# gwlucastrig/gridfour

Hardware: AMD Instinct MI355X
Metric: encode+decode MB/s on int32 elevation tiles; bit-exact vs Java ref (higher is better)
Workload: dtype int32

## Files before the change

gridfour_amd/csrc/gvrs_decode.hip:

```cpp

#include <hip/hip_runtime.h>

#include <cstdlib>
#include <mutex>
#include <type_traits>

#include "gvrs_kernels.h"
#include "huff_build.h"

namespace {

constexpr int GF_K_SKIP = 0x7fff0001;
#ifndef GF_DEC_THREADS
#define GF_DEC_THREADS 256
#endif
#ifdef GF_DEC_VARIANT
#define GF_DEC_CAT2(a, b) a##b
#define GF_DEC_CAT(a, b) GF_DEC_CAT2(a, b)
#define gf_launch_huffman_decode GF_DEC_CAT(gf_launch_huffman_decode_t, GF_DEC_THREADS)
#define gf_huffman_decode_lds_per_wg GF_DEC_CAT(gf_huffman_decode_lds_per_wg_t, GF_DEC_THREADS)
#define gf_launch_huffman_decode_canon GF_DEC_CAT(gf_launch_huffman_decode_canon_t, GF_DEC_THREADS)
#endif
constexpr int DEC_THREADS = GF_DEC_THREADS;
constexpr int DEC_WAVES = DEC_THREADS / 64;
// ... 557 lines not shown
                if (cnt[i] & 3u) *reinterpret_cast<uint32_t *>(poolB + slot[i]) = lo[i];
                if (d[i] && cnt[i] > 4u * poolWords) S.poolOverflow = 1u;
            }
        }
#pragma unroll
        for (int i = 0; i < NCUR; i++)
            if (d[i]) { S.qs[qv[i]] = sPos[i]; S.qe[qv[i]] = a[i] - sh0; S.qn[qv[i]] = cnt[i]; }
    };
#ifdef GF_DIAG
    const uint32_t tBegin = (uint32_t)__builtin_amdgcn_s_memtime();
#endif
    {
        uint32_t qv[NCUR];
#pragma unroll
        for (int i = 0; i < NCUR; i++) qv[i] = tid + i * DEC_THREADS;
        runRound(true, qv);
    }
#ifdef GF_DIAG
    if (dbg && tid == 0) dbg[1] = (uint32_t)__builtin_amdgcn_s_memtime() - tBegin;
#endif
    for (uint32_t round = 1;; round++) {
        __syncthreads();
#ifdef GF_DIAG
        rounds++;
        if (dbg && tid == 0 && round == 1) dbg[3] = (uint32_t)__builtin_amdgcn_s_memtime() - tBegin;
#endif
        if (tid == 0) S.nRedo[(round + 1u) & 1u] = 0;
#pragma unroll
        for (int i = 0; i < NCUR; i++) {
            const uint32_t q = tid + i * DEC_THREADS;
            if (q > 0 && q < Q && S.qe[q - 1] != S.qs[q]) {
                const uint32_t slot = atomicAdd(&S.nRedo[round & 1u], 1u);
                if (slot < LIST_CAP) list[slot] = (uint16_t)q;
            }
        }
        __syncthreads();
        const uint32_t nList = min(S.nRedo[round & 1u], LIST_CAP);
        if (nList == 0) break;
#ifdef GF_DIAG
        listed += nList;
#endif
        uint32_t qv[NCUR];
#pragma unroll
        for (int i = 0; i < NCUR; i++) {
            const uint32_t slot = gf_wave_id() * (64u * NCUR) + (uint32_t)i * 64u + (tid & 63u);
            qv[i] = slot < nList ? list[slot] : 0xFFFFFFFFu;
        }
        runRound(false, qv);
    }
    uint32_t n[NCUR], sum = 0;
#pragma unroll
    for (int i = 0; i < NCUR; i++) {
        const uint32_t q = NCUR * tid + i;
        n[i] = q < Q ? S.qn[q] : 0u;
        sum += n[i];
    }
    uint32_t tot;
    uint32_t run = block_excl_scan(sum, S.waveSum, &tot);
#pragma unroll
    for (int i = 0; i < NCUR; i++) {
        const uint32_t q = NCUR * tid + i;
        if (q < Q) S.qn[q] = run;
        run += n[i];
    }
    if (tid == 0) S.chainTotal = tot;
#ifdef GF_DIAG
    if (dbg && tid == 0) { dbg[0] = rounds; dbg[DBG_LISTED] = listed; dbg[4] = (uint32_t)__builtin_amdgcn_s_memtime() - tBegin; }
#endif
    __syncthreads();
}

struct RCur {
    uint32_t pos, sh, r0, r1, r2, r3, r4, r5, r6, r7;
};
__device__ __forceinline__ void rcur_load(RCur &c, const uint32_t *__restrict__ base32, uint32_t nW, uint32_t sh0, uint32_t p)
{
    const uint32_t a = p + sh0, wi = a >> 5;
    c.pos = p;
    c.sh = a & 31u;
    if (wi + 8u <= nW) {
        const GfU4 x = *reinterpret_cast<const GfU4 *>(base32 + wi), y = *reinterpret_cast<const GfU4 *>(base32 + wi + 4);
        c.r0 = x.x; c.r1 = x.y; c.r2 = x.z; c.r3 = x.w;
        c.r4 = y.x; c.r5 = y.y; c.r6 = y.z; c.r7 = y.w;
    } else {
        const uint32_t last = nW - 1u;
        c.r0 = base32[min(wi, last)];
        c.r1 = base32[min(wi + 1u, last)];
        c.r2 = base32[min(wi + 2u, last)];
        c.r3 = base32[min(wi + 3u, last)];
        c.r4 = base32[min(wi + 4u, last)];
        c.r5 = base32[min(wi + 5u, last)];
        c.r6 = base32[min(wi + 6u, last)];
        c.r7 = base32[min(wi + 7u, last)];
    }
}
__device__ __forceinline__ void rcur_advance(RCur &c, uint32_t len)
{
    c.pos += len;
    const uint32_t sh = c.sh + len;
    const bool ge = sh >= 32u;
    c.r0 = ge ? c.r1 : c.r0;
    c.r1 = ge ? c.r2 : c.r1;
    c.r2 = ge ? c.r3 : c.r2;
    c.r3 = ge ? c.r4 : c.r3;
    c.r4 = ge ? c.r5 : c.r4;
    c.r5 = ge ? c.r6 : c.r5;
    c.r6 = ge ? c.r7 : c.r6;
    c.sh = sh & 31u;
}
constexpr uint32_t RCUR_BUDGET = 256u - 31u - 96u;

__device__ __forceinline__ void pool_to_m32(DecShared &S, const uint32_t *pool, uint32_t poolWords, uint32_t Q, uint32_t nM32, uint8_t *m32,
                                            uint32_t spare)
{
    const uint32_t tid = threadIdx.x;
    uint32_t *m32w = reinterpret_cast<uint32_t *>(m32);
#pragma unroll
    for (int i = 0; i < NCUR; i++) {
        const uint32_t q = tid + (uint32_t)i * DEC_THREADS;
        uint32_t base = 0, n = 0;
        if (q < Q) {
            base = S.qn[q];
            n = (q + 1u < Q ? S.qn[q + 1u] : S.chainTotal) - base;
            n = base < nM32 ? min(n, nM32 - base) : 0u;
        }
        const uint32_t *src = pool + (q < Q ? q : 0u);
        const uint32_t h = min(n, (0u - base) & 3u);
        const uint32_t nb = (n - h) >> 2, r = (n - h) & 3u;
        const uint32_t w0 = (base + h) >> 2;
        uint32_t tailWord = 0, first = 0;
        for (uint32_t c = 0; c < poolWords; c += 8u) {
            if (!__any(4u * c < n)) break;
            uint32_t w[9];
#pragma unroll
            for (uint32_t j = 0; j < 9u; j++) w[j] = c + j < poolWords ? src[(c + j) * Q] : 0u;
            if (c == 0u) first = w[0];
#pragma unroll
            for (uint32_t j = 0; j < 8u; j++) {
                const uint32_t k = c + j;
                const uint32_t out = __builtin_amdgcn_alignbyte(w[j + 1u], w[j], h);
                m32w[k < nb ? w0 + k : spare >> 2] = out;
                tailWord = k == nb ? out : tailWord;
            }
        }
#pragma unroll
        for (uint32_t j = 0; j < 3u; j++) {
            m32[j < h ? base + j : spare] = (uint8_t)(first >> (8u * j));
            m32[j < r ? base + h + 4u * nb + j : spare] = (uint8_t)(tailWord >> (8u * j));
        }
    }
}

template <int OWNER>
__device__ int32_t huffman_to_m32_fast(DecShared &S, const uint32_t *__restrict__ base32, uint32_t nW, uint32_t sh0,
                                       uint32_t *txt, uint32_t pkWords, const uint16_t *lut2, const unsigned long long *leafCodeG,
                                       uint32_t textStart, uint32_t endBit, uint32_t nM32, uint8_t *m32, uint32_t *dbg,
                                       const uint32_t warmBits, const int diagLimit = 0, uint32_t *pool = nullptr, uint32_t poolBytes = 0,
                                       uint32_t spareByte = 0)
{
    const uint32_t tid = threadIdx.x;
    int32_t status = GF_K_OK;
    const uint32_t textBits = endBit - textStart;
    uint32_t unit = (textBits + MAXQ - 1) / MAXQ;
    unit = max((uint32_t)GF_DEC_MIN_UNIT, (unit + 31u) & ~31u);
    const uint32_t Q = max(1u, (textBits + unit - 1) / unit);
    FastHuff H;
    H.S = &S;
    H.lut2 = lut2;
    H.leafCodeG = leafCodeG;
    H.l2bits = S.l2bits;
    H.nSub = S.nSub;
    uint16_t *cnt16 = reinterpret_cast<uint16_t *>(S.leafCode);
    static_assert(sizeof(S.leafCode) >= (sizeof(uint16_t) << LUT_BITS), "count table does not fit over leafCode");
    build_count_table(S, cnt16);
#ifdef GF_DIAG
    const uint32_t tStage = (uint32_t)__builtin_amdgcn_s_memtime();
#endif
    for (uint32_t i = tid + (uint32_t)EARLY_TXT * DEC_THREADS; i < pkWords + FAST_TEXT_PAD; i += DEC_THREADS) txt[i] = (i < pkWords && i < nW) ? base32[i] : 0u;
    __syncthreads();
#ifdef GF_DIAG
    if (dbg && tid == 0) dbg[2] = (uint32_t)__builtin_amdgcn_s_memtime() - tStage;
#endif
#ifdef GF_DIAG
    if (diagLimit == 7) return GF_K_SKIP;
#endif
    uint32_t poolWords = pool ? min(33u, (poolBytes / Q) >> 2) : 0u;
    poolWords = poolWords < 17u ? 0u : poolWords - 1u;
    fast_sync_pass<OWNER>(S, H, cnt16, txt, sh0, textStart, endBit, unit, Q, warmBits, dbg, poolWords ? pool : nullptr, poolWords);
#ifdef GF_DIAG
    if (diagLimit == 8) return GF_K_SKIP;
    if (dbg && tid == 0) dbg[-7] = (uint32_t)__builtin_amdgcn_s_memtime();
#else
    (void)dbg;
#endif
    if (S.chainTotal < nM32) status = GF_K_ERR_BOUNDS;
#ifdef GF_DEC_POOL_FORCE_OVERFLOW
    if (false) {
#else
    if (poolWords && !S.poolOverflow) {
#endif
        pool_to_m32(S, pool, poolWords, Q, nM32, m32, spareByte);
        if (status == GF_K_OK && S.chainTotal == nM32 && S.qe[Q - 1u] > endBit) status = GF_K_ERR_BOUNDS;
        __syncthreads();
        return status;
    }
    if (tid == 0) S.chainEnd = 0;
    __syncthreads();
    {
        bool d[NCUR];
        uint32_t k[NCUR], lim[NCUR];
        RCur c[NCUR];
#pragma unroll
        for (int i = 0; i < NCUR; i++) {
            const uint32_t q = tid + i * DEC_THREADS;
            d[i] = q < Q;
            k[i] = d[i] ? S.qn[q] : nM32;
            lim[i] = min(endBit, textStart + (q + 1) * unit);
            c[i].pos = d[i] ? S.qs[q] : endBit;
        }
        for (;;) {
            bool live[NCUR], anyLive = false;
#pragma unroll
            for (int i = 0; i < NCUR; i++) {
                live[i] = d[i] && c[i].pos < lim[i] && k[i] < nM32;
                anyLive = anyLive || live[i];
            }
            if (!__any(anyLive)) break;
            uint32_t blk[NCUR];
#pragma unroll
            for (int i = 0; i < NCUR; i++) {
                rcur_load(c[i], base32, nW, sh0, live[i] ? c[i].pos : 0u);
                if (!live[i]) c[i].pos = endBit;
                blk[i] = c[i].pos;
            }
            for (;;) {
                bool r[NCUR], any = false;
#pragma unroll
                for (int i = 0; i < NCUR; i++) {
                    r[i] = live[i] && c[i].pos < lim[i] && k[i] < nM32 && c[i].pos - blk[i] <= RCUR_BUDGET;
                    any = any || r[i];
                }
                if (!__any(any)) break;
                uint32_t x[NCUR], e[NCUR], anyLong = 0;
#pragma unroll
                for (int i = 0; i < NCUR; i++) {
                    x[i] = __builtin_amdgcn_alignbit(c[i].r1, c[i].r0, c[i].sh);
                    e[i] = S.lut[x[i] & ((1u << LUT_BITS) - 1u)];
                    anyLong |= e[i];
                }
                if (anyLong & 0x80000000u) {
#pragma unroll
                    for (int i = 0; i < NCUR; i++)
                        if (e[i] & 0x80000000u) e[i] = fh_resolve(H, e[i], x[i], c[i].r0, c[i].r1, c[i].r2, c[i].sh);
                }
#pragma unroll
                for (int i = 0; i < NCUR; i++) {
                    const uint32_t a1 = (e[i] >> 16) & 63u, t2 = e[i] >> 22;
                    const bool two = t2 != a1 && c[i].pos + a1 < lim[i] && nM32 - k[i] > 1u;
                    rcur_advance(c[i], r[i] ? (two ? t2 : a1) : 0u);
                    if (r[i]) {
                        m32[k[i]] = (uint8_t)e[i];
                        if (two) m32[k[i] + 1] = (uint8_t)(e[i] >> 8);
                        k[i] += two ? 2u : 1u;
                        if (k[i] == nM32) S.chainEnd = c[i].pos;
                    }
                }
            }
        }
    }
    __syncthreads();
    if (status == GF_K_OK && S.chainEnd > endBit) status = GF_K_ERR_BOUNDS;
    return status;
}


__device__ __forceinline__ int gf_writelane(int value, int lane, int old)
{
    return (int)(threadIdx.x & 63u) == lane ? value : old;
}

__device__ void parse_tree_wave(DecShared &S, uint32_t relBit, uint32_t absBit, uint32_t totalBits)
{
    const uint32_t lane = threadIdx.x & 63u;
    const uint32_t hw0 = S.head[lane];
    const uint32_t hw1 = lane < HEAD_WORDS - 64 ? S.head[64 + lane] : 0u;
    auto word = [&](uint32_t wi) -> uint32_t {
        if (wi >= HEAD_WORDS) return 0u;
        return (uint32_t)__builtin_amdgcn_readlane((int)(wi < 64 ? hw0 : hw1), (int)(wi & 63u));
    };
    const uint32_t fw = relBit >> 5, fs = relBit & 31u;
    uint64_t buf = (((uint64_t)word(fw + 1u) << 32) | word(fw)) >> fs;
    uint32_t have = 64u - fs, wnext = fw + 2u, bp = absBit;
    auto refill = [&]() {
        if (have <= 32) {
            buf |= (uint64_t)word(wnext) << have;
            have += 32;
            wnext++;
        }
    };
    auto take = [&](uint32_t nb) -> uint32_t {
        const uint32_t v = (uint32_t)buf & ((1u << nb) - 1u);
        buf >>= nb;
        have -= nb;
        bp += nb;
        return v;
    };
    const bool writer = lane == 0;
// ... 919 lines not shown

constexpr uint32_t BYTE_MAX_COLS = 256;
__device__ __forceinline__ bool byte_path_eligible(int model, uint32_t nR, uint32_t nC, uint32_t ldsM32Bytes)
{
    const uint32_t RB = (nR + DEC_WAVES - 1u) / DEC_WAVES;
    return model >= 1 && model <= 3 && nR >= 2u && nC >= 4u && nC <= BYTE_MAX_COLS && RB <= 255u && nR * nC + 8u <= ldsM32Bytes &&
           ((2u * nR + 3u) & ~3u) + (model == 3 ? (uint32_t)DEC_WAVES * ((nC + 3u) & ~3u) : 0u) <= SCR_WORDS;
}

template <int MODEL>
__device__ __forceinline__ void m32_bytes_rows(DecShared &S, const uint8_t *m32, const uint32_t seed, const uint32_t nR, const uint32_t nC,
                                               uint32_t *__restrict__ o)
{
    const uint32_t lane = threadIdx.x & 63u, wave = gf_wave_id();
    uint32_t *scr = reinterpret_cast<uint32_t *>(&S);
    uint32_t *col0 = scr, *d1s = scr + nR, *T = scr + ((2u * nR + 3u) & ~3u);
    const uint32_t TS = (nC + 3u) & ~3u;
    const uint32_t *m32w = reinterpret_cast<const uint32_t *>(m32);
    const uint32_t j0 = 4u * lane;
    const uint32_t jf = j0 < nC ? j0 : 0u;
    auto sx = [](uint32_t b) -> uint32_t { return (uint32_t)(int32_t)(int8_t)b; };
    if (wave == (uint32_t)DEC_WAVES - 1u) {
        uint32_t carry = seed;
        for (uint32_t rb = 0; rb < nR; rb += 64u) {
            const uint32_t r = rb + lane;
            uint32_t x = 0;
            if (r >= 1u && r < nR) x = sx(m32[MODEL == 3 ? nC - 2u + r : MODEL == 1 ? r * nC - 1u : 2u * r - 1u]);
            const uint32_t v = gf_wave_incl_scan(x) + carry;
            if (r < nR) col0[r] = v;
            carry = (uint32_t)__builtin_amdgcn_readlane((int)v, 63);
        }
    } else if (MODEL == 2 && wave == (uint32_t)DEC_WAVES - 2u) {
        for (uint32_t r = lane; r < nR; r += 64u) d1s[r] = sx(m32[2u * r]);
    }
    const uint32_t RB = (nR + DEC_WAVES - 1u) / DEC_WAVES;
    const uint32_t r0 = min(nR, wave * RB), r1 = min(nR, r0 + RB);
    const uint32_t rowStep = MODEL == 1 ? nC : MODEL == 2 ? nC - 2u : nC - 1u;
    auto rowAt = [&](uint32_t r) -> uint32_t {
        if (MODEL == 1) return r * nC - 1u;
        if (MODEL == 2) return 2u * nR - 1u + r * (nC - 2u) - 2u;
        return r ? nC + nR - 2u + (r - 1u) * (nC - 1u) - 1u : 0u - 1u;
    };
    auto fetch = [&](uint32_t a4) -> uint32_t {
        const uint32_t wi = a4 >> 2;
        return __builtin_amdgcn_alignbyte(m32w[wi], m32w[wi - 1u], a4 & 3u);
    };
    auto fetchRow0 = [&]() -> uint32_t { return __builtin_amdgcn_alignbyte(m32w[lane], lane ? m32w[lane - 1u] : 0u, 3u); };
    const bool peel = MODEL != 2 && r0 == 0u && r1 > 0u;
    const uint32_t keep0 = lane == 0u ? 0u : 0xFFFFFFFFu;
    uint32_t acc0 = 0, acc1 = 0, acc2 = 0, acc3 = 0;
    if (MODEL == 3) {
        if (wave + 1u < (uint32_t)DEC_WAVES && r1 > r0) {
            uint32_t ev = 0, od = 0;
            uint32_t r = r0;
            if (peel) {
                const uint32_t y = fetchRow0() ^ 0x80808080u;
                ev = y & 0x00FF00FFu;
                od = (y >> 8) & 0x00FF00FFu;
                r = 1u;
            }
            uint32_t a4 = rowAt(r) + jf + 4u;
            for (; r < r1; r++) {
                const uint32_t y = fetch(a4) ^ 0x80808080u;
                ev += y & 0x00FF00FFu;
                od += (y >> 8) & 0x00FF00FFu;
                a4 += rowStep;
            }
            const uint32_t bias = 128u * (r1 - r0);
            const uint32_t c0 = ((ev & 0xFFFFu) - bias) & keep0, c1 = (od & 0xFFFFu) - bias, c2 = (ev >> 16) - bias, c3 = (od >> 16) - bias;
            const uint32_t p1 = c0 + c1, p2 = p1 + c2, p3 = p2 + c3;
            const uint32_t ex = gf_wave_incl_scan(p3) - p3;
            if (j0 < TS) {
                uint32_t *Tw = T + wave * TS + j0;
                Tw[0] = ex + c0; Tw[1] = ex + p1; Tw[2] = ex + p2; Tw[3] = ex + p3;
            }
        }
    }
    __syncthreads();
    if (MODEL == 3 && j0 < TS) {
        for (uint32_t w = 0; w < wave; w++) {
            const uint32_t *Tw = T + w * TS + j0;
            acc0 += Tw[0]; acc1 += Tw[1]; acc2 += Tw[2]; acc3 += Tw[3];
        }
    }
    const uint32_t nFull = nC >> 2, rem = nC & 3u;
    const bool full = lane < nFull, part = lane == nFull && rem != 0u;
    struct Quad { uint32_t q0, q1, q2, q3; };
    auto sums = [&](uint32_t x, uint32_t left, uint32_t d1) -> Quad {
        const uint32_t v0 = sx(x) & keep0, v1 = MODEL == 2 ? sx(x >> 8) & keep0 : sx(x >> 8), v2 = sx(x >> 16), v3 = (uint32_t)((int32_t)x >> 24);
        const uint32_t p1 = v0 + v1, p2 = p1 + v2, p3 = p2 + v3;
        const uint32_t ex = gf_wave_incl_scan(p3) - p3;
        Quad q;
        if (MODEL == 2) {
            const uint32_t g1 = v0 + p1, g2 = g1 + p2, g3 = g2 + p3;
            const uint32_t t = g3 + 4u * ex;
            const uint32_t gx = gf_wave_incl_scan(t) - t;
            const uint32_t b = left + j0 * d1 + gx + ex;
            q.q0 = b + v0;
            q.q1 = b + d1 + ex + g1;
            q.q2 = b + 2u * (d1 + ex) + g2;
            q.q3 = b + 3u * (d1 + ex) + g3;
        } else if (MODEL == 3) {
            acc0 += ex + v0; acc1 += ex + p1; acc2 += ex + p2; acc3 += ex + p3;
            q.q0 = acc0 + left; q.q1 = acc1 + left; q.q2 = acc2 + left; q.q3 = acc3 + left;
        } else {
            const uint32_t b = left + ex;
            q.q0 = b + v0; q.q1 = b + p1; q.q2 = b + p2; q.q3 = b + p3;
        }
        return q;
    };
    auto put = [&](uint32_t r, const Quad &q) {
        uint32_t *dst = o + r * nC + j0;
        if (full) {
            GfU4 v;
            v.x = q.q0; v.y = q.q1; v.z = q.q2; v.w = q.q3;
            *reinterpret_cast<GfU4 *>(dst) = v;
        }
        if (part) {
            dst[0] = q.q0;
            if (rem >= 2u) dst[1] = q.q1;
            if (rem == 3u) dst[2] = q.q2;
        }
    };
    uint32_t r = r0;
    if (peel) {
        put(0u, sums(fetchRow0(), col0[0], 0u));
        r = 1u;
    }
    if (r < r1) {
        const uint32_t last = r1 - 1u;
        uint32_t a4 = rowAt(r) + jf + 4u, rB = min(r + 1u, last);
        uint32_t a4B = a4 + (rB - r) * rowStep;
        uint32_t xA = fetch(a4), leftA = col0[r], dA = MODEL == 2 ? d1s[r] : 0u;
        uint32_t xB = fetch(a4B), leftB = col0[rB], dB = MODEL == 2 ? d1s[rB] : 0u;
        for (; r < r1; r += 2u) {
            const uint32_t x0 = xA, l0 = leftA, e0 = dA, x1 = xB, l1 = leftB, e1 = dB;
            const uint32_t nA = min(r + 2u, last), nB = min(r + 3u, last);
            a4 += (nA - r) * rowStep;
            a4B = a4 + (nB - nA) * rowStep;
            xA = fetch(a4);
            leftA = col0[nA];
            xB = fetch(a4B);
            leftB = col0[nB];
            if (MODEL == 2) { dA = d1s[nA]; dB = d1s[nB]; }
            const Quad qa = sums(x0, l0, e0);
            const Quad qb = sums(x1, l1, e1);
            put(r, qa);
            if (r + 1u < r1) put(r + 1u, qb);
        }
    }
    __syncthreads();
}

template <class M32Ptr>
__device__ __forceinline__ void m32_bytes_to_tile(DecShared &S, M32Ptr m32, const int model, const uint32_t seed, const uint32_t nR,
                                                  const uint32_t nC, uint32_t *__restrict__ o)
{
    if (model == 3) m32_bytes_rows<3>(S, m32, seed, nR, nC, o);
    else if (model == 1) m32_bytes_rows<1>(S, m32, seed, nR, nC, o);
    else m32_bytes_rows<2>(S, m32, seed, nR, nC, o);
}

template <class M32Ptr>
__device__ int32_t huffman_serial_skips(DecShared &S, const uint32_t *__restrict__ base32, uint32_t nW, uint32_t sh0, uint32_t textStart,
                                        uint32_t endBit, uint32_t nM32, M32Ptr m32)
{
    const uint32_t tid = threadIdx.x, lane = tid & 63u;
    if (tid < 64u) {
        const uint32_t nLeaves = S.nLeaves;
        unsigned long long lc[4];
        uint32_t ll[4], ls[4];
#pragma unroll
        for (uint32_t j = 0; j < 4; j++) {
            const uint32_t i = lane + 64u * j;
            lc[j] = i < nLeaves ? S.leafCode[i] : 0ull;
            ll[j] = i < nLeaves ? (uint32_t)S.leafLen[i] : 0xFFu;
            ls[j] = i < nLeaves ? (uint32_t)S.leafSym[i] : 0u;
        }
        const uint32_t skipLen = GF_UNI(S.skipLen);
        const unsigned long long skipPath = ((unsigned long long)GF_UNI(S.skipHi) << 32) | GF_UNI(S.skipLo);
        uint32_t pos = textStart, k = 0;
        int32_t st = GF_K_OK;
        while (k < nM32) {
            unsigned long long cur = 0;
            uint32_t len = 0;
            bool emitted = false, restart = false;
            while (!emitted && !restart) {
                if (pos >= endBit || len >= 64u) { st = GF_K_ERR_BOUNDS; break; }
                const uint32_t g = pos + sh0, wi = g >> 5;
                const uint32_t w = wi < nW ? GF_UNI(base32[wi]) : 0u;
                const uint32_t b = (w >> (g & 31u)) & 1u;
                pos++;
                cur |= (unsigned long long)b << len;
                len++;
                bool hit = false;
                uint32_t sym = 0;
#pragma unroll
                for (uint32_t j = 0; j < 4; j++)
                    if (ll[j] == len && lc[j] == cur) { hit = true; sym = ls[j]; }
                const unsigned long long m = __ballot(hit);
                if (m) {
                    const uint32_t who = (uint32_t)__builtin_ctzll(m);
                    const uint32_t v = (uint32_t)__builtin_amdgcn_readlane((int)sym, (int)who);
                    if (lane == 0u) m32[k] = (uint8_t)v;
                    k++;
                    emitted = true;
                } else if (len <= skipLen && b == 1u && ((skipPath >> (len - 1u)) & 1ull) == 0ull &&
                           ((cur ^ skipPath) & ((1ull << (len - 1u)) - 1ull)) == 0ull) {
                    restart = true;
                }
            }
            if (st != GF_K_OK) break;
        }
        if (lane == 0u) {
            S.chainEnd = pos;
            S.chainTotal = k;
            S.parseStatus = st;
        }
    }
    __syncthreads();
    const int32_t st = S.parseStatus;
    __syncthreads();
    return st;
}

#ifdef GF_DIAG
#define GF_DSTAMP(i)                                                                   \
    do {                                                                               \
        if (a.debug && tid == 0) (a.debug + t * 16)[i] = (uint32_t)__builtin_amdgcn_s_memtime(); \
    } while (0)
#define GF_DPHASE_LIMIT(n, what) \
    if ((a.phaseLimit & 0xff) == (n)) what
#else
#define GF_DSTAMP(i) do { } while (0)
#define GF_DPHASE_LIMIT(n, what)
#endif

constexpr int GF_K_RETRY = 0x7fff0002;

enum { DEC_GENERAL = 0, DEC_ANALYZE = 1, DEC_FAST = 2, DEC_FAST_ROOMY = 3, DEC_FAST_CANON = 4 };

template <int MODE>
__global__ __launch_bounds__(DEC_THREADS, MODE >= 2 ? GF_DEC_WGS : GF_DEC_WGS_GENERAL) void k_huffman_decode(GfDecodeArgs a)
{
    __shared__ DecShared S;
    extern __shared__ __attribute__((aligned(16))) uint8_t ldsDyn[];
    constexpr bool ANALYZE = MODE == DEC_ANALYZE;
    constexpr bool ROOMY = MODE == DEC_FAST_ROOMY;
    constexpr bool CANON = MODE == DEC_FAST_CANON;
    constexpr bool FAST = MODE == DEC_FAST || ROOMY || CANON;
    constexpr int OWNER = MODE;

    const int tid = threadIdx.x, wave = (int)gf_wave_id();
    const uint32_t nR = (uint32_t)a.nRows, nC = (uint32_t)a.nCols, nCells = nR * nC;
    const uint32_t *__restrict__ w32 = reinterpret_cast<const uint32_t *>(a.blob);
    const uint64_t nWords = (a.blobBytes + 3) >> 2;
    if constexpr (MODE == DEC_GENERAL) {
        if (a.retryFlag && a.ldsM32Roomy && blockIdx.x == 0 && tid == 0) {
            if (a.roomySeenHost) *a.roomySeenHost = 1u + a.retryFlag[2];
            a.retryFlag[2] = 0u;
            a.retryFlag[3] = 0u;
        }
        if (a.retryFlag && a.retryFlag[a.ldsM32Roomy ? 1 : 0] == 0u) return;
    }
    auto roomy_next = [&]() -> size_t {
        __syncthreads();
        if (tid == 0) S.carry = atomicAdd(a.retryFlag + 3, 1u);
        __syncthreads();
        const uint32_t i = S.carry;
        return i < min(a.retryFlag[2], (uint32_t)a.nTiles) ? (size_t)a.roomyList[i] : ~(size_t)0;
    };

    for (size_t t = ROOMY ? roomy_next() : (size_t)blockIdx.x + (size_t)blockIdx.y * gridDim.x; t < a.nTiles;
         t = ROOMY ? roomy_next() : (MODE == DEC_FAST || CANON) ? ~(size_t)0 : t + gridDim.x) {
        if constexpr (MODE == DEC_GENERAL) {
            if (a.retryFlag && a.status[t] != GF_K_RETRY) continue;
        }
        const uint64_t off = a.offsets ? a.offsets[t] : (uint64_t)t * a.slotStride;
        const uint32_t len = a.lengths[t];
        uint32_t *o = reinterpret_cast<uint32_t *>(a.values) + t * (size_t)nCells;
        const uint8_t *__restrict__ pk = a.blob + off;
        constexpr bool PRE = FAST;
        unsigned long long preCode = 0;
        uint32_t preLen = 0, preSym = 0, preRec[8] = {0, 0, 0, 0, 0, 0, 0, 0};
        uint32_t preHead = 0;
        const bool headEarly = PRE && off + 12u <= a.blobBytes;
        if constexpr (PRE && CANON) {
            if (headEarly && tid < 12) preHead = pk[tid];
            const uint32_t *recP = a.trees + t * GF_CANON_REC_WORDS;
            preRec[0] = recP[0];
            preRec[1] = recP[1];
            if (tid < 256) preLen = reinterpret_cast<const uint8_t *>(recP + 8)[tid];
            if (tid < 16) preSym = reinterpret_cast<const uint8_t *>(recP + 8)[256 + tid];
        } else if constexpr (PRE) {
            if (headEarly && tid < 12) preHead = pk[tid];
            const uint32_t *recP = a.trees + t * GF_TREE_REC_WORDS;
#pragma unroll
            for (int i = 0; i < 8; i++) preRec[i] = recP[i];
            if (tid < 256) {
                preCode = reinterpret_cast<const unsigned long long *>(recP + 8)[tid];
                preLen = reinterpret_cast<const uint8_t *>(recP + 8 + 512)[tid];
                preSym = reinterpret_cast<const uint8_t *>(recP + 8 + 512 + 64)[tid];
            }
        }

        auto canon_leave = [&]() {
            if (tid == 0) {
                a.status[t] = GF_K_RETRY;
                atomicOr(a.retryFlag, 1u);
            }
// ... 224 lines not shown
                    S.skipHi = R(7);
                    S.textStart = R(2);
                    S.parseStatus = (int32_t)R(0);
                    S.nLeaves = nLeaves;
                }
                S.nShort = nShort;
                S.l2bits = l2;
                S.nSub = min(nSub, (uint32_t)L2_ENTRIES >> l2);
                S.maxLen = maxLen;
            }
        } else if (wave == 0) {
            if constexpr (!FAST) parse_tree_wave(S, 80u, 80u, len * 8u);
        }
        __syncthreads();
        if (S.parseStatus != GF_K_OK) {
            if (tid == 0) {
                a.status[t] = S.parseStatus;
                if constexpr (CANON) atomicOr(a.retryFlag, 1u);
            }
            __syncthreads();
            continue;
        }
        if constexpr (FAST) {
            const uint32_t pkWords = (((uint32_t)(off * 8ull) & 31u) + len * 8u + 31u) >> 5;
            if (S.maxLen > 32u || S.skipLen != 0u || (pkWords + FAST_TEXT_PAD) * 4u > a.ldsM32Bytes) {
                if (tid == 0) {
                    a.status[t] = GF_K_RETRY;
                    atomicOr(a.retryFlag + (a.ldsM32Roomy ? 1 : 0), 1u);
                }
                __syncthreads();
                continue;
            }
        }
        GF_DSTAMP(2);
        GF_DPHASE_LIMIT(1, continue);
#ifdef GF_DIAG
        const uint32_t warmBits = (a.phaseLimit >> 8) ? (uint32_t)(a.phaseLimit >> 8) : 128u;
        uint32_t *const dbg = a.debug ? a.debug + t * 16 + 11 : nullptr;
#else
        constexpr uint32_t warmBits = 128u;
        constexpr uint32_t *dbg = nullptr;
#endif

        const size_t bmRaw = 2 * (((size_t)a.ldsM32Bytes >> 5) + 2) * 4;
        const size_t bmArea = bmRaw > 2 * L2_ENTRIES ? bmRaw : 2 * L2_ENTRIES;
        uint16_t *lut2 = reinterpret_cast<uint16_t *>(ldsDyn + a.ldsM32Bytes);
        bool fused = false;
        auto phases12 = [&](auto inLds) -> int32_t {
            uint8_t *m32;
            uint32_t *bm, *wb;
            if constexpr (decltype(inLds)::value) {
                m32 = ldsDyn;
                bm = reinterpret_cast<uint32_t *>(ldsDyn + a.ldsM32Bytes);
                wb = bm + (a.ldsM32Bytes >> 5) + 1;
            } else {
                uint8_t *ws = a.workspace + (size_t)blockIdx.x * a.workspaceStride;
                m32 = ws;
                const size_t cap = ((size_t)6 * nCells + 31) & ~(size_t)31;
                bm = reinterpret_cast<uint32_t *>(ws + cap);
                wb = bm + (cap >> 5) + 1;
            }
            int32_t tileStatus = GF_K_OK;

            if (!FAST && a.rawM32) {
                for (uint32_t i = tid; i < nM32; i += DEC_THREADS) m32[i] = pk[10 + i];
                __syncthreads();
            } else if (S.uniformSym >= 0) {
                const uint8_t sym = (uint8_t)S.uniformSym;
                for (uint32_t i = tid; i < nM32; i += DEC_THREADS) m32[i] = sym;
                __syncthreads();
            } else if (!FAST && S.skipLen != 0u) {
                const uint64_t baseWord = (off * 8ull) >> 5;
                tileStatus = huffman_serial_skips(S, w32 + baseWord, (uint32_t)min((uint64_t)0xffffffffu, nWords - baseWord),
                                                  (uint32_t)(off * 8ull) & 31u, S.textStart, len * 8u, nM32, m32);
            } else {
                build_lut(S, lut2);
                GF_DSTAMP(3);
                GF_DPHASE_LIMIT(6, return (int32_t)GF_K_SKIP);
                const uint32_t textStart = S.textStart, endBit = len * 8u;
                const uint64_t baseWord = (off * 8ull) >> 5;
                const uint32_t sh0 = (uint32_t)(off * 8ull) & 31u;
                const uint32_t pkWords = (sh0 + endBit + 31u) >> 5;
                if constexpr (FAST) {
                    tileStatus = huffman_to_m32_fast<OWNER>(S, w32 + baseWord, (uint32_t)min((uint64_t)0xffffffffu, nWords - baseWord),
                                                           sh0, reinterpret_cast<uint32_t *>(ldsDyn), pkWords, lut2,
                                                           reinterpret_cast<const unsigned long long *>(CANON ? a.trees : a.trees + t * GF_TREE_REC_WORDS + 8),
#ifdef GF_DIAG
                                                           textStart, endBit, nM32, m32, dbg, warmBits, a.phaseLimit & 0xff,
#else
                                                           textStart, endBit, nM32, m32, dbg, warmBits, 0,
#endif
                                                           a.lean ? nullptr : o, nCells * 4u, a.ldsM32Bytes + 4u);
                } else if (pkWords * 4u <= a.ldsTextBytes) {
                    uint32_t *txt = reinterpret_cast<uint32_t *>(ldsDyn + a.ldsM32Bytes + bmArea);
                    const uint64_t avail = nWords - baseWord;
                    for (uint32_t i = tid; i < pkWords; i += DEC_THREADS) txt[i] = i < avail ? w32[baseWord + i] : 0u;
                    __syncthreads();
                    HuffCursorT<const uint32_t *> cur;
                    cur.base32 = txt;
                    cur.nW = pkWords;
                    cur.sh0 = sh0;
                    cur.S = &S;
                    cur.lut2 = lut2;
                    tileStatus = huffman_to_m32<OWNER>(S, cur, textStart, endBit, nM32, m32, dbg, warmBits);
                } else {
                    HuffCursorT<const uint32_t *> cur;
                    cur.base32 = w32 + baseWord;
                    cur.nW = (uint32_t)min((uint64_t)0xffffffffu, nWords - baseWord);
                    cur.sh0 = sh0;
                    cur.S = &S;
                    cur.lut2 = lut2;
                    tileStatus = huffman_to_m32<OWNER>(S, cur, textStart, endBit, nM32, m32, dbg, warmBits);
                }
            }
            if (tileStatus != GF_K_OK) return tileStatus;
            GF_DSTAMP(5);
            GF_DPHASE_LIMIT(2, return (int32_t)GF_K_SKIP);
            if constexpr (ANALYZE) {
                uint32_t *hist = S.lut;
                for (uint32_t i = tid; i < 256; i += DEC_THREADS) hist[i] = 0;
                __syncthreads();
                for (uint32_t i = tid; i < nM32; i += DEC_THREADS) atomicAdd(&hist[m32[i]], 1u);
                if (a.pairCounts && nM32 >= 2u) {
                    uint32_t *pc = a.pairCounts + (size_t)(model >= 0 && model < GF_PAIR_TABLES ? model : 0) * 65536u;
                    for (uint32_t i = tid + 1u; i < nM32; i += DEC_THREADS) atomicAdd(&pc[((uint32_t)m32[i - 1u] << 8) | m32[i]], 1u);
                }
                __syncthreads();
                uint32_t *rec = a.analysis + t * GF_ANALYSIS_WORDS;
                if (tid == 0) {
                    rec[0] = (uint32_t)model;
                    rec[1] = nM32;
                    rec[2] = S.textStart - 80u;
                    rec[3] = len - 10u;
                    a.status[t] = GF_K_OK;
                }
                for (uint32_t i = tid; i < 256; i += DEC_THREADS) rec[4 + i] = hist[i];
                __syncthreads();
                return (int32_t)GF_K_SKIP;
            } else {
                if constexpr (CANON && decltype(inLds)::value) {
                    const uint32_t eb = S.skipLo, eb4 = eb * 0x01010101u;
                    const uint32_t *mw = reinterpret_cast<const uint32_t *>(m32);
                    uint32_t bad = 0;
                    for (uint32_t i = tid; 4u * i < nStream; i += DEC_THREADS) {
                        const uint32_t v = mw[i] ^ eb4;
                        uint32_t z = ~(((v & 0x7F7F7F7Fu) + 0x7F7F7F7Fu) | v) & 0x80808080u;
                        const uint32_t left = nStream - 4u * i;
                        if (left < 4u) z &= (1u << (8u * left)) - 1u;
                        bad |= z;
                    }
                    if (tid == 0 && m32[nStream] != (uint8_t)eb) bad = 1u;
                    if (__syncthreads_or((int)(bad != 0u))) return (int32_t)GF_K_RETRY;
                    fused = true;
                    m32_bytes_to_tile(S, m32, model, seed, nR, nC, o);
                    return (int32_t)GF_K_OK;
                }
                if constexpr (FAST && !CANON && decltype(inLds)::value) {
                    if (!(GF_UNI(S.symKinds) & (GF_TREE_HAS_INTRODUCER | GF_TREE_HAS_NULL)) && byte_path_eligible(model, nR, nC, a.ldsM32Bytes)) {
                        fused = true;
                        GF_DPHASE_LIMIT(4, return (int32_t)GF_K_OK);
                        m32_bytes_to_tile(S, m32, model, seed, nR, nC, o);
                        return (int32_t)GF_K_OK;
                    }
                }
                if constexpr (decltype(inLds)::value) {
                    if (FAST || (plan.ring && model >= 1 && model <= 3)) {
                        fused = true;
                        #ifdef GF_DIAG
                        return m32_to_tile(S, m32, nM32, bm, wb, model, seed, nR, nC, nStream, plan, o, dbg ? dbg - 11 : nullptr, (uint32_t)a.phaseLimit);
#else
                        return m32_to_tile(S, m32, nM32, bm, wb, model, seed, nR, nC, nStream, plan, o, nullptr, 0u);
#endif
                    }
                }
                if constexpr (!FAST) {
                    const CellMapPredictor map{GfCellMap::make(model, nR, nC)};
                    tileStatus = m32_to_values(S, m32, nM32, bm, wb, nStream, map, o);
                }
                return tileStatus;
            }
        };
        int32_t tileStatus;
        if constexpr (FAST) tileStatus = phases12(std::true_type{});
        else tileStatus = nM32 <= a.ldsM32Bytes ? phases12(std::true_type{}) : phases12(std::false_type{});
        if (tileStatus == (int32_t)GF_K_SKIP) continue;
        if constexpr (CANON) {
            if (tileStatus != GF_K_OK) {
                canon_leave();
                continue;
            }
        }
        if (tileStatus != GF_K_OK) {
            if (tid == 0) a.status[t] = tileStatus;
            __syncthreads();
            continue;
        }
        GF_DSTAMP(8);
        GF_DPHASE_LIMIT(3, continue);

        if constexpr (!FAST) {
            if (!fused) gf_predictor_inverse(model, seed, o, nR, nC, nullptr);
        }
        GF_DSTAMP(10);
        if (tid == 0) a.status[t] = GF_K_OK;
        __syncthreads();
    }
}

#ifndef GF_DEC_VARIANT
__global__ __launch_bounds__(DEC_THREADS, 4) void k_lsop_unpack_m32(GfLsopM32Args a)
{
    __shared__ DecShared S;
    extern __shared__ __attribute__((aligned(16))) uint8_t ldsDyn[];

    const int tid = threadIdx.x, wave = (int)gf_wave_id();
    const uint32_t nR = (uint32_t)a.nRows, nC = (uint32_t)a.nCols, nCells = nR * nC;
    const uint32_t nInit = 4u * nR + 2u * nC - 9u, nInt = (nR - 2u) * (nC - 4u);
    const uint32_t *__restrict__ w32 = reinterpret_cast<const uint32_t *>(a.blob);
    const uint64_t nWords = (a.blobBytes + 3) >> 2;

    for (size_t t = blockIdx.x; t < a.nTiles; t += gridDim.x) {
        if (a.status[t] != GF_K_ERR_UNSUPPORTED) continue;
        const uint64_t off = a.offsets ? a.offsets[t] : (uint64_t)t * a.slotStride;
        const uint32_t len = a.lengths[t];
        const uint8_t *__restrict__ pk = a.blob + off;
        uint32_t *res = reinterpret_cast<uint32_t *>(a.residuals) + t * a.resStride;
        auto le32 = [&](uint32_t o) -> uint32_t {
            return (uint32_t)pk[o] | ((uint32_t)pk[o + 1] << 8) | ((uint32_t)pk[o + 2] << 16) | ((uint32_t)pk[o + 3] << 24);
        };

        int32_t early = GF_K_OK;
        uint32_t o = 1, type = 0, nMI = 0, nMX = 0;
        bool checksum = false;
        if (len < 3 || off + len > a.blobBytes) early = GF_K_ERR_BOUNDS;
        else {
            const bool revised = pk[1] & 0x40;
            if (revised) { type = pk[1] & 0x0fu; checksum = pk[1] & 0x80; o = 2; }
            if (len < o + 1u + 52u + 8u + (revised ? 0u : 1u)) early = GF_K_ERR_BOUNDS;
            else if (pk[o] != 12) early = GF_K_ERR_FORMAT;
            else {
                o += 53;
                nMI = le32(o);
                nMX = le32(o + 4);
                o += 8;
                if (!revised) { type = pk[o] & 0x0fu; checksum = pk[o] & 0x80; o++; }
                if (checksum) o += 4;
                if (o > len) early = GF_K_ERR_BOUNDS;
                else if (type == 2) early = GF_K_ERR_UNSUPPORTED;
                else if (type != 0 && !a.rawM32) early = GF_K_ERR_UNSUPPORTED;
                else if (nMI > 6u * nInit + 64u || nMX > 6u * nInt + 64u) early = GF_K_ERR_FORMAT;
                else if (type != 0 && a.rawM32 == 1 && (uint64_t)o + nMI + nMX > len) early = GF_K_ERR_BOUNDS;
                else if (type != 0 && a.rawM32 == 2) {
                    const int32_t sd = a.sideStatus[t];
                    if (sd < 0) early = sd;
                    else if (sd != 0) early = GF_K_ERR_UNSUPPORTED;
                    else if (a.inflStatus2[t] != GF_K_OK || a.produced2[t] < nMX) early = GF_K_ERR_FORMAT;
                }
            }
        }
        if (early != GF_K_OK) {
            if (tid == 0) a.status[t] = early;
            __syncthreads();
            continue;
        }
        if (tid < 13) a.coefs[t * 16 + tid] = le32((pk[1] & 0x40 ? 3u : 2u) + 4u * tid);

        uint32_t startBit = o * 8u;
        uint32_t rawAt = a.rawM32 == 2 ? 0u : o;
        const uint8_t *__restrict__ rawFrom = a.rawM32 == 2 ? a.rawSide + t * a.rawSideStride : pk;
        int32_t tileStatus = GF_K_OK;
        for (int seg = 0; seg < 2 && tileStatus == GF_K_OK; seg++) {
            const uint32_t nM32 = seg ? nMX : nMI, nVals = seg ? nInt : nInit;
            uint32_t *out = res + (seg ? nInit : 0u);
            auto segment = [&](auto inLds) -> int32_t {
                uint8_t *m32;
                uint32_t *bm, *wb;
                if constexpr (decltype(inLds)::value) {
                    m32 = ldsDyn;
                    bm = reinterpret_cast<uint32_t *>(ldsDyn + a.ldsM32Bytes);
                    wb = bm + (a.ldsM32Bytes >> 5) + 1;
                } else {
                    uint8_t *ws = a.workspace + (size_t)blockIdx.x * a.workspaceStride;
                    m32 = ws;
                    const size_t cap = ((size_t)6 * nCells + 31) & ~(size_t)31;
                    bm = reinterpret_cast<uint32_t *>(ws + cap);
                    wb = bm + (cap >> 5) + 1;
                }
                if (type != 0) {
                    for (uint32_t i = tid; i < nM32; i += DEC_THREADS) m32[i] = rawFrom[rawAt + i];
                    __syncthreads();
                } else {
                    const uint32_t hb0 = (startBit >> 5) << 2;
                    {
                        uint8_t *hb = reinterpret_cast<uint8_t *>(S.head);
                        for (uint32_t i = tid; i < HEAD_WORDS * 4; i += DEC_THREADS) hb[i] = hb0 + i < len ? pk[hb0 + i] : 0;
                    }
                    __syncthreads();
                    if (wave == 0) parse_tree_wave(S, startBit & 31u, startBit, len * 8u);
                    __syncthreads();
                    if (S.parseStatus != GF_K_OK) return S.parseStatus;
                    if (S.uniformSym >= 0) {
                        const uint8_t sym = (uint8_t)S.uniformSym;
                        for (uint32_t i = tid; i < nM32; i += DEC_THREADS) m32[i] = sym;
                        if (tid == 0) S.chainEnd = S.textStart;
                        __syncthreads();
                    } else if (S.skipLen != 0u) {
                        const uint64_t baseWord = (off * 8ull) >> 5;
                        const int32_t st = huffman_serial_skips(S, w32 + baseWord, (uint32_t)min((uint64_t)0xffffffffu, nWords - baseWord),
                                                                (uint32_t)(off * 8ull) & 31u, S.textStart, len * 8u, nM32, m32);
                        if (st != GF_K_OK) return st;
                        if (nM32 == 0 && tid == 0) S.chainEnd = S.textStart;
                        __syncthreads();
                    } else {
                        uint16_t *lut2 = reinterpret_cast<uint16_t *>(ldsDyn + a.ldsM32Bytes);
// ... 622 lines not shown
```

Baseline: 805,800.

## Add half-wave byte-to-tile reconstruction with K cells per lane

Adds a new byte-stream-to-tile reconstruction path in which each 32-lane half-wave handles its own row band and each lane owns five consecutive columns. Row prefix sums use in-register scans combined with a DPP half-wave scan, and model 3 column carries go through cross-wave LDS partial sums. This is meant to raise parallelism and row throughput for tiles up to 160 columns compared with the existing one-row-per-wave path. The path is used for canonical tiles and for non-roomy fast tiles when scratch fits. It also forces inlining of huffman_to_m32_fast, which may raise register pressure.

```diff
diff --git a/gridfour_amd/csrc/gvrs_decode.hip b/gridfour_amd/csrc/gvrs_decode.hip
--- a/gridfour_amd/csrc/gvrs_decode.hip
+++ b/gridfour_amd/csrc/gvrs_decode.hip
@@ -733,7 +733,7 @@
 }
 
 template <int OWNER>
-__device__ int32_t huffman_to_m32_fast(DecShared &S, const uint32_t *__restrict__ base32, uint32_t nW, uint32_t sh0,
+__device__ __forceinline__ int32_t huffman_to_m32_fast(DecShared &S, const uint32_t *__restrict__ base32, uint32_t nW, uint32_t sh0,
                                        uint32_t *txt, uint32_t pkWords, const uint16_t *lut2, const unsigned long long *leafCodeG,
                                        uint32_t textStart, uint32_t endBit, uint32_t nM32, uint8_t *m32, uint32_t *dbg,
                                        const uint32_t warmBits, const int diagLimit = 0, uint32_t *pool = nullptr, uint32_t poolBytes = 0,
@@ -1959,10 +1959,234 @@
     __syncthreads();
 }
 
+constexpr uint32_t BYTE_HALF_SLACK = 16;
+constexpr uint32_t BYTE_HALF_K = 5, BYTE_HALF_MAX_COLS = 32u * BYTE_HALF_K;
+__device__ __forceinline__ bool byte_half_fits(int model, uint32_t nR, uint32_t nC, uint32_t ldsM32Bytes)
+{
+    const uint32_t TS = (nC + BYTE_HALF_K - 1u) / BYTE_HALF_K * BYTE_HALF_K;
+    return nC <= BYTE_HALF_MAX_COLS && nR * nC + BYTE_HALF_SLACK <= ldsM32Bytes &&
+           ((2u * nR + 3u) & ~3u) + (model == 3 ? ((uint32_t)DEC_WAVES - 1u) * TS : 0u) <= SCR_WORDS;
+}
+
+__device__ __forceinline__ uint32_t gf_half_incl_scan(uint32_t v)
+{
+#if defined(__HIP_DEVICE_COMPILE__)
+    int x = (int)v;
+    x += __builtin_amdgcn_update_dpp(0, x, 0x111, 0xf, 0xf, true);
+    x += __builtin_amdgcn_update_dpp(0, x, 0x112, 0xf, 0xf, true);
+    x += __builtin_amdgcn_update_dpp(0, x, 0x114, 0xf, 0xf, true);
+    x += __builtin_amdgcn_update_dpp(0, x, 0x118, 0xf, 0xf, true);
+    x += __builtin_amdgcn_update_dpp(0, x, 0x142, 0xa, 0xf, false);
+    return (uint32_t)x;
+#else
+    return v;
+#endif
+}
+
+template <int K>
+struct __attribute__((packed, aligned(4))) GfCells {
+    uint32_t c[K];
+};
+
+template <int MODEL, int K>
+__device__ __forceinline__ void m32_bytes_rows_half(DecShared &S, const uint8_t *m32, const uint32_t seed, const uint32_t nR,
+                                                    const uint32_t nC, uint32_t *__restrict__ o)
+{
+    static_assert(K >= 5 && K <= 8, "a lane's bytes are two aligned words");
+    constexpr uint32_t NB = 2u * (uint32_t)DEC_WAVES;
+    const uint32_t lane = threadIdx.x & 63u, wave = gf_wave_id();
+    const uint32_t half = lane >> 5, hl = lane & 31u;
+    uint32_t *scr = reinterpret_cast<uint32_t *>(&S);
+    uint32_t *col0 = scr, *d1s = scr + nR, *T = scr + ((2u * nR + 3u) & ~3u);
+    const uint32_t nFull = nC / (uint32_t)K, rem = nC - nFull * (uint32_t)K;
+    const uint32_t TS = (nFull + (rem ? 1u : 0u)) * (uint32_t)K;
+    const uint32_t *m32w = reinterpret_cast<const uint32_t *>(m32);
+    const uint32_t j0 = (uint32_t)K * hl;
+    const uint32_t jf = j0 < nC ? j0 : 0u;
+    auto sx = [](uint32_t b) -> uint32_t { return (uint32_t)(int32_t)(int8_t)b; };
+    if (wave == (uint32_t)DEC_WAVES - 1u) {
+        uint32_t carry = seed;
+        for (uint32_t rb = 0; rb < nR; rb += 64u) {
+            const uint32_t r = rb + lane;
+            uint32_t x = 0;
+            if (r >= 1u && r < nR) x = sx(m32[MODEL == 3 ? nC - 2u + r : MODEL == 1 ? r * nC - 1u : 2u * r - 1u]);
+            const uint32_t v = gf_wave_incl_scan(x) + carry;
+            if (r < nR) col0[r] = v;
+            carry = (uint32_t)__builtin_amdgcn_readlane((int)v, 63);
+        }
+    } else if (MODEL == 2 && wave == (uint32_t)DEC_WAVES - 2u) {
+        for (uint32_t r = lane; r < nR; r += 64u) d1s[r] = sx(m32[2u * r]);
+    }
+    const uint32_t RBH = (nR + NB - 1u) / NB;
+    const uint32_t w0 = min(nR, 2u * wave * RBH), n0 = min(nR, w0 + RBH) - w0;
+    const uint32_t r0 = half ? min(nR, w0 + RBH) : w0, r1 = min(nR, r0 + RBH), nh = r1 - r0;
+    const uint32_t rS = min(r0, nR - 1u), lastF = max(max(r1, rS + 1u) - 1u, 1u);
+    const uint32_t rowStep = MODEL == 1 ? nC : MODEL == 2 ? nC - 2u : nC - 1u;
+    auto rowAt = [&](uint32_t r) -> uint32_t {
+        if (MODEL == 1) return r * nC - 1u;
+        if (MODEL == 2) return 2u * nR - 1u + r * (nC - 2u) - 2u;
+        return r ? nC + nR - 2u + (r - 1u) * (nC - 1u) - 1u : 0u - 1u;
+    };
+    struct Bytes { uint32_t lo, hi; };
+    auto fetch = [&](uint32_t a4) -> Bytes {
+        const uint32_t wi = a4 >> 2, m = m32w[wi];
+        Bytes b;
+        b.lo = __builtin_amdgcn_alignbyte(m, m32w[wi - 1u], a4 & 3u);
+        b.hi = __builtin_amdgcn_alignbyte(m32w[wi + 1u], m, a4 & 3u);
+        return b;
+    };
+    auto fetchAny = [&](uint32_t a4) -> Bytes {
+        const uint32_t wi = a4 >> 2, m = m32w[wi];
+        Bytes b;
+        b.lo = __builtin_amdgcn_alignbyte(m, m32w[wi ? wi - 1u : 0u], a4 & 3u);
+        b.hi = __builtin_amdgcn_alignbyte(m32w[wi + 1u], m, a4 & 3u);
+        return b;
+    };
+    const uint32_t keep0 = hl == 0u ? 0u : 0xFFFFFFFFu;
+    const uint32_t a4Last = rowAt(lastF) + jf + 4u;
+    const uint32_t rSB = min(rS + 1u, lastF);
+    uint32_t acc[K];
+#pragma unroll
+    for (int i = 0; i < K; i++) acc[i] = 0;
+    if (MODEL == 3) {
+        uint32_t evL = 0, odL = 0, evH = 0, odH = 0;
+        auto add = [&](const Bytes &b) {
+            const uint32_t yl = b.lo ^ 0x80808080u, yh = b.hi ^ 0x80808080u;
+            evL += yl & 0x00FF00FFu;
+            odL += (yl >> 8) & 0x00FF00FFu;
+            evH += yh & 0x00FF00FFu;
+            odH += (yh >> 8) & 0x00FF00FFu;
+        };
+        const uint32_t rP = min(r0, nR - n0);
+        if (n0 > 0u) add(fetchAny(rowAt(rP) + jf + 4u));
+        uint32_t a4 = rowAt(rP + 1u) + jf + 4u;
+        for (uint32_t i = 1; i < n0; i++) {
+            add(fetch(a4));
+            a4 += rowStep;
+        }
+        const uint32_t bias = 128u * n0;
+        uint32_t c[8];
+        c[0] = ((evL & 0xFFFFu) - bias) & keep0; c[1] = (odL & 0xFFFFu) - bias; c[2] = (evL >> 16) - bias; c[3] = (odL >> 16) - bias;
+        c[4] = (evH & 0xFFFFu) - bias; c[5] = (odH & 0xFFFFu) - bias; c[6] = (evH >> 16) - bias; c[7] = (odH >> 16) - bias;
+#pragma unroll
+        for (int i = 1; i < K; i++) c[i] += c[i - 1];
+        const uint32_t ex = gf_half_incl_scan(c[K - 1]) - c[K - 1];
+        uint32_t other[K];
+#pragma unroll
+        for (int i = 0; i < K; i++) {
+            c[i] += ex;
+            other[i] = (uint32_t)__shfl_xor((int)c[i], 32, 64);
+            if (half) acc[i] = other[i];
+        }
+        if (!half && j0 < TS && wave + 1u < (uint32_t)DEC_WAVES) {
+            uint32_t *Tw = T + wave * TS + j0;
+#pragma unroll
+            for (int i = 0; i < K; i++) Tw[i] = c[i] + other[i];
+        }
+    }
+    __syncthreads();
+    if (MODEL == 3 && j0 < TS) {
+        for (uint32_t w = 0; w < wave; w++) {
+            const uint32_t *Tw = T + w * TS + j0;
+#pragma unroll
+            for (int i = 0; i < K; i++) acc[i] += Tw[i];
+        }
+    }
+    const bool hasPart = rem != 0u;
+    const uint32_t fullRows = hl < nFull ? nh : 0u, partRows = hl == nFull ? nh : 0u;
+    struct Cells { uint32_t q[K]; };
+    auto sums = [&](const Bytes &x, uint32_t left, uint32_t d1) -> Cells {
+        uint32_t v[K], p[K];
+#pragma unroll
+        for (int i = 0; i < K; i++) {
+            const uint32_t w = i < 4 ? x.lo : x.hi;
+            v[i] = (i & 3) == 3 ? (uint32_t)((int32_t)w >> 24) : sx(w >> (8 * (i & 3)));
+        }
+        v[0] &= keep0;
+        if (MODEL == 2) v[1] &= keep0;
+        p[0] = v[0];
+#pragma unroll
+        for (int i = 1; i < K; i++) p[i] = p[i - 1] + v[i];
+        const uint32_t ex = gf_half_incl_scan(p[K - 1]) - p[K - 1];
+        Cells q;
+        if (MODEL == 2) {
+            uint32_t g[K];
+            g[0] = p[0];
+#pragma unroll
+            for (int i = 1; i < K; i++) g[i] = g[i - 1] + p[i];
+            const uint32_t t = g[K - 1] + (uint32_t)K * ex;
+            const uint32_t gx = gf_half_incl_scan(t) - t;
+            const uint32_t b = left + j0 * d1 + gx + ex, s = d1 + ex;
+#pragma unroll
+            for (int i = 0; i < K; i++) q.q[i] = b + (uint32_t)i * s + g[i];
+        } else if (MODEL == 3) {
+#pragma unroll
+            for (int i = 0; i < K; i++) {
+                acc[i] += ex + p[i];
+                q.q[i] = acc[i] + left;
+            }
+        } else {
+            const uint32_t b = left + ex;
+#pragma unroll
+            for (int i = 0; i < K; i++) q.q[i] = b + p[i];
+        }
+        return q;
+    };
+    auto put = [&](uint32_t off, const Cells &q, uint32_t i) {
+        uint32_t *dst = o + off;
+        if (i < fullRows) {
+            GfCells<K> v;
+#pragma unroll
+            for (int k = 0; k < K; k++) v.c[k] = q.q[k];
+            *reinterpret_cast<GfCells<K> *>(dst) = v;
+        }
+        if (hasPart) {
+            if (i < partRows) {
+                dst[0] = q.q[0];
+#pragma unroll
+                for (int k = 1; k < K - 1; k++)
+                    if (rem > (uint32_t)k) dst[k] = q.q[k];
+            }
+        }
+    };
+    if (n0 > 0u) {
+        uint32_t off = r0 * nC + j0;
+        uint32_t cA = rS, cB = rSB, a4B = rowAt(rSB) + jf + 4u;
+        Bytes xA = fetchAny(rowAt(rS) + jf + 4u), xB = fetchAny(a4B);
+        uint32_t leftA = col0[cA], leftB = col0[cB], dA = MODEL == 2 ? d1s[cA] : 0u, dB = MODEL == 2 ? d1s[cB] : 0u;
+        for (uint32_t i = 0; i < n0; i += 2u) {
+            const Bytes x0 = xA, x1 = xB;
+            const uint32_t l0 = leftA, e0 = dA, l1 = leftB, e1 = dB;
+            const uint32_t a4A = min(a4B + rowStep, a4Last);
+            a4B = min(a4A + rowStep, a4Last);
+            cA = min(cB + 1u, lastF);
+            cB = min(cA + 1u, lastF);
+            xA = fetch(a4A);
+            leftA = col0[cA];
+            xB = fetch(a4B);
+            leftB = col0[cB];
+            if (MODEL == 2) { dA = d1s[cA]; dB = d1s[cB]; }
+            const Cells qa = sums(x0, l0, e0);
+            const Cells qb = sums(x1, l1, e1);
+            put(off, qa, i);
+            put(off + nC, qb, i + 1u);
+            off += 2u * nC;
+        }
+    }
+    __syncthreads();
+}
+
 template <class M32Ptr>
 __device__ __forceinline__ void m32_bytes_to_tile(DecShared &S, M32Ptr m32, const int model, const uint32_t seed, const uint32_t nR,
-                                                  const uint32_t nC, uint32_t *__restrict__ o)
-{
+                                                  const uint32_t nC, const bool halfForm, const uint32_t ldsM32Bytes,
+                                                  uint32_t *__restrict__ o)
+{
+    if (halfForm && byte_half_fits(model, nR, nC, ldsM32Bytes)) {
+        if (model == 3) m32_bytes_rows_half<3, BYTE_HALF_K>(S, m32, seed, nR, nC, o);
+        else if (model == 1) m32_bytes_rows_half<1, BYTE_HALF_K>(S, m32, seed, nR, nC, o);
+        else m32_bytes_rows_half<2, BYTE_HALF_K>(S, m32, seed, nR, nC, o);
+        return;
+    }
     if (model == 3) m32_bytes_rows<3>(S, m32, seed, nR, nC, o);
     else if (model == 1) m32_bytes_rows<1>(S, m32, seed, nR, nC, o);
     else m32_bytes_rows<2>(S, m32, seed, nR, nC, o);
@@ -2493,14 +2717,14 @@
                     if (tid == 0 && m32[nStream] != (uint8_t)eb) bad = 1u;
                     if (__syncthreads_or((int)(bad != 0u))) return (int32_t)GF_K_RETRY;
                     fused = true;
-                    m32_bytes_to_tile(S, m32, model, seed, nR, nC, o);
+                    m32_bytes_to_tile(S, m32, model, seed, nR, nC, true, a.ldsM32Bytes, o);
                     return (int32_t)GF_K_OK;
                 }
                 if constexpr (FAST && !CANON && decltype(inLds)::value) {
                     if (!(GF_UNI(S.symKinds) & (GF_TREE_HAS_INTRODUCER | GF_TREE_HAS_NULL)) && byte_path_eligible(model, nR, nC, a.ldsM32Bytes)) {
                         fused = true;
                         GF_DPHASE_LIMIT(4, return (int32_t)GF_K_OK);
-                        m32_bytes_to_tile(S, m32, model, seed, nR, nC, o);
+                        m32_bytes_to_tile(S, m32, model, seed, nR, nC, !ROOMY, a.ldsM32Bytes, o);
                         return (int32_t)GF_K_OK;
                     }
                 }
```

New measurement: 810,700 (median of 6 runs). No clear change (+0.6%).
